# liannuaa/GenPC

Hardware: NVIDIA B200
Metric: chamfer_fwd_bwd_point_pairs_per_sec (higher is better)
Workload: dtype f32

## Files before the change

genpc_b200/csrc/chamfer.cu:

```cuda
#include <cstdlib>
#include <cstring>
#include <mutex>
#include <new>

#include "nn_core.cuh"
#include "nn_sym.cuh"
#include "nn_tc.cuh"
#include "nn_prune.cuh"
#include "nn_grid.cuh"

#ifndef GENPC_DEFAULT_SYM
#define GENPC_DEFAULT_SYM true
#endif
#ifndef GENPC_DEFAULT_PERSIST
#define GENPC_DEFAULT_PERSIST false
#endif
#ifndef GENPC_DEFAULT_BALANCED
#define GENPC_DEFAULT_BALANCED true
#endif

namespace genpc {

struct NNDir {
    const float *q;
// ... 283 lines not shown
    int cs = 1, mixed = 0;
    const char *k = tunable("GENPC_SORT_CLUSTER");
    if (k != nullptr) {
        mixed = k[0] == 'm' ? 1 : 0;
        cs = atoi(k + mixed);
        cs = cs >= 8 ? 8 : cs >= 4 ? 4 : cs == 3 ? 3 : cs == 2 ? 2 : 1;
    } else if (nmax >= 8192) {
        if (nmin * 4 <= nmax && nmin <= 4096) {
            mixed = 1;
            cs = nb * 4 + (nb + 3) / 4 * 4 <= sms ? 4 : nb * 3 + (nb + 2) / 3 * 3 <= sms ? 3 : nb * 2 + (nb + 1) / 2 * 2 <= sms ? 2 : 1;
        } else {
            cs = nb * 16 <= sms ? 8 : nb * 8 <= sms ? 4 : nb * 4 <= sms ? 2 : 1;
        }
    }
    if (cs < 2) mixed = 0;
    const int ctas = mixed ? nb * cs + nb : 2 * nb * cs;
    *mixed_out = mixed;
    *grid_out = (ctas + cs - 1) / cs * cs;
    return cs;
}

static void launch_bin_sort(PruneSortParams sp, int nb, cudaStream_t stream) {
    int mixed = 0, grid = 0;
    const int cs = sort_layout(nb, sp.n[0], sp.n[1], num_sms(), &mixed, &grid);
    sp.mixed = mixed;
    const int ctas = mixed ? nb * cs + nb : 2 * nb * cs;
    if (cs == 8) launch_bin_sort_cs<8>(sp, ctas, stream);
    else if (cs == 4) launch_bin_sort_cs<4>(sp, ctas, stream);
    else if (cs == 3) launch_bin_sort_cs<3>(sp, ctas, stream);
    else if (cs == 2) launch_bin_sort_cs<2>(sp, ctas, stream);
    else nn_bin_sort_kernel<1><<<2 * nb, PR_SORT_THREADS, 0, stream>>>(sp);
}

static int launch_prune_subbatch(const float *rows, const float *cols, int nr, int nc, unsigned long long *prow, unsigned long long *pcol,
                                 int B, int b0, int nb, int *ctl, void *prune_extra, bool accumulate, cudaStream_t stream,
                                 int *chunk_ctl = nullptr) {
    char *w = reinterpret_cast<char *>((reinterpret_cast<size_t>(prune_extra) + 255) & ~(size_t)255);
    float4 *sorted0 = reinterpret_cast<float4 *>(w);
    float4 *sorted1 = sorted0 + (size_t)B * pr_npad(nr);
    float4 *boxes0 = sorted1 + (size_t)B * pr_npad(nc);
    float4 *boxes1 = boxes0 + (size_t)B * 2 * pr_nblk(nr);
    float *bbx = reinterpret_cast<float *>(boxes1 + (size_t)B * 2 * pr_nblk(nc));
    PruneSortParams sp = {};
    sp.xyz[0] = rows + (size_t)b0 * nr * 3, sp.xyz[1] = cols + (size_t)b0 * nc * 3, sp.n[0] = nr, sp.n[1] = nc, sp.B = nb;
    sp.limit = 1e15f, sp.ctl = chunk_ctl != nullptr ? chunk_ctl : ctl, sp.hilbert = 1, sp.accumulate = accumulate ? 1 : 0;
    sp.flag = chunk_ctl != nullptr ? ctl + 1 : nullptr;
    sp.sorted[0] = sorted0 + (size_t)b0 * pr_npad(nr), sp.sorted[1] = sorted1 + (size_t)b0 * pr_npad(nc);
    sp.boxes[0] = boxes0 + (size_t)b0 * 2 * pr_nblk(nr), sp.boxes[1] = boxes1 + (size_t)b0 * 2 * pr_nblk(nc);
    sp.bbx = bbx + (size_t)b0 * 16;
    launch_bin_sort(sp, nb, stream);
    GENPC_CHECK_LAUNCH();
    PruneParams q = {};
    q.B = nb, q.select = ctl + 1, q.stats = g_prune_stats;
    q.q = sp.sorted[0], q.t = sp.sorted[1], q.tbox = sp.boxes[1], q.out = prow + (size_t)b0 * nr, q.nq = nr, q.nt = nc;
    PruneParams q2 = q;
    q2.q = sp.sorted[1], q2.t = sp.sorted[0], q2.tbox = sp.boxes[0], q2.out = pcol + (size_t)b0 * nc, q2.nq = nc, q2.nt = nr;
    launch_prune(q, q2, stream);
    GENPC_CHECK_LAUNCH();
    return GENPC_OK;
}

static int chamfer_forward_sym(const float *xyz1, const float *xyz2, float *dist1, float *dist2, int *idx1, int *idx2,
                               int B, int N, int M, unsigned long long *packed, int *counter, cudaStream_t stream,
                               const unsigned *gate = nullptr, unsigned gate_gen = 0, int gate_pairs = 1,
                               const genpc_chamfer_fuse_t *fuse = nullptr, double *fuse_partial = nullptr,
                               unsigned *fuse_ticket = nullptr, void *prune_extra = nullptr, const int *prune_chunks = nullptr) {
    const bool swap = M > N;
    SymParams p = {};
    p.rows = swap ? xyz2 : xyz1, p.cols = swap ? xyz1 : xyz2;
    p.nr = swap ? M : N, p.nc = swap ? N : M;
    float *dist_r = swap ? dist2 : dist1, *dist_c = swap ? dist1 : dist2;
    int *idx_r = swap ? idx2 : idx1, *idx_c = swap ? idx1 : idx2;
    p.prow = packed, p.pcol = packed + (size_t)B * p.nr;
    p.rblock_base = 0;
    p.gate = gate, p.gate_gen = gate_gen, p.gate_pairs = gate_pairs;
    p.select = nullptr;
    int *ctl = counter;
    const bool use_grid = ctl != nullptr && gate == nullptr && prune_extra != nullptr && B <= 8 && grid_eligible(p.nr, p.nc);
    const bool use_prune = use_grid || (ctl != nullptr && gate == nullptr && prune_extra != nullptr && prune_eligible(B, p.nr, p.nc));
    if (use_grid) {
        char *w = reinterpret_cast<char *>((reinterpret_cast<size_t>(prune_extra) + 255) & ~(size_t)255);
        GridParams gp = {};
        gp.B = B, gp.limit = 1e15f, gp.ctl = ctl;
        gp.xyz[0] = p.rows, gp.xyz[1] = p.cols, gp.n[0] = p.nr, gp.n[1] = p.nc;
        for (int i = 0; i < 2; ++i) {
            gp.sorted[i] = reinterpret_cast<float4 *>(w), w += (size_t)B * pr_npad(gp.n[i]) * sizeof(float4);
            gp.boxes[i] = reinterpret_cast<float4 *>(w), w += (size_t)B * 2 * pr_nblk(gp.n[i]) * sizeof(float4);
            gp.sboxes[i] = reinterpret_cast<float4 *>(w), w += (size_t)B * 2 * gr_nsb(gp.n[i]) * sizeof(float4);
        }
// ... 19 lines not shown
                                                                 (const int *)vals_in, vals_out, gp.n[side], 0, 30, stream);
                if (es != cudaSuccess) return (int)es;
                grid_gather_kernel<<<ctas, GR_THREADS, 0, stream>>>(gp, side, b, side == 0 && b == 0);
            }
        GENPC_CHECK_LAUNCH();
        const int nblk_max = pr_nblk(nmax), nsb_max = gr_nsb(nmax);
        grid_boxes_kernel<false><<<dim3((nblk_max + 7) / 8, B, 2), GR_THREADS, 0, stream>>>(gp);
        grid_boxes_kernel<true><<<dim3((nsb_max + 7) / 8, B, 2), GR_THREADS, 0, stream>>>(gp);
        GENPC_CHECK_LAUNCH();
        p.select = ctl + 1;
        Prune2Params q = {};
        q.B = B, q.select = ctl + 1, q.stats = g_prune_stats;
        const char *pk = tunable("GENPC_CHAMFER_PRUNE");
        const bool forced = pk != nullptr && atoi(pk) == 2;
        for (int pass = forced ? 1 : 0; pass < 2; ++pass) {
            const bool probe = pass == 0;
            long long limit = 0;
            for (int dir = 0; dir < 2; ++dir) {
                q.q = gp.sorted[dir], q.t = gp.sorted[1 - dir], q.tbox = gp.boxes[1 - dir], q.tsbox = gp.sboxes[1 - dir];
                q.out = dir == 0 ? p.prow : p.pcol, q.nq = gp.n[dir], q.nt = gp.n[1 - dir];
                const int groups = (q.nq + PR_GROUP - 1) / PR_GROUP, nblk = pr_nblk(q.nt);
                q.probe_stride = groups > GR_PROBE_GROUPS ? groups / GR_PROBE_GROUPS : 1;
                q.probe_cap = nblk / 5 > 64 ? nblk / 5 : 64;
                q.probe_acc = ctl + 2;
                const long long sampled = (long long)B * ((groups + q.probe_stride - 1) / q.probe_stride);
                limit += sampled * (nblk / 10 > 16 ? nblk / 10 : 16);
                launch_prune2(q, stream, probe);
            }
            if (probe) grid_decide_kernel<<<1, 1, 0, stream>>>(ctl, (int)(limit > 0x7fffffffLL ? 0x7fffffffLL : limit));
        }
        GENPC_CHECK_LAUNCH();
    } else if (use_prune) {
        if (prune_chunks == nullptr) {
            const int rcp = launch_prune_subbatch(p.rows, p.cols, p.nr, p.nc, p.prow, p.pcol, B, 0, B, ctl, prune_extra, false, stream);
            if (rcp != GENPC_OK) return rcp;
        } else {
            prune_rearm_kernel<<<2 * GENPC_NUM_SMS, 256, 0, stream>>>(p.prow, (size_t)B * (p.nr + p.nc), ctl + 1);
            GENPC_CHECK_LAUNCH();
        }
        p.select = ctl + 1;
    }
    const bool use_tc = !use_prune && ctl != nullptr && tc_eligible(B, p.nr, p.nc);
    if (use_tc) {
        static bool attr_done = false;
        if (!attr_done) {
            cudaError_t ea = cudaFuncSetAttribute(nn_tc_kernel<false>, cudaFuncAttributeMaxDynamicSharedMemorySize, (int)sizeof(TcSmem));
            if (ea == cudaSuccess) ea = cudaFuncSetAttribute(nn_tc_kernel<true>, cudaFuncAttributeMaxDynamicSharedMemorySize, (int)sizeof(TcSmem));
            if (ea != cudaSuccess) return (int)ea;
            attr_done = true;
        }
        const char *lim = tunable("GENPC_TC_LIMIT");
        const float limit = lim != nullptr ? (float)atof(lim) : 2.0f;
        if (gate == nullptr) {
            nn_tc_precheck_kernel<<<2 * GENPC_NUM_SMS, 256, 0, stream>>>(p.rows, (size_t)B * p.nr * 3, p.cols, (size_t)B * p.nc * 3, limit, ctl);
            GENPC_CHECK_LAUNCH();
            p.select = ctl + 1;
        }
        TcParams t = {};
        t.rows = p.rows, t.cols = p.cols, t.prow = p.prow, t.pcol = p.pcol, t.B = B, t.nr = p.nr, t.nc = p.nc;
        t.rblks = (p.nr + TC_RBLK - 1) / TC_RBLK, t.total_units = B * t.rblks;
        t.select = p.select, t.gate = gate, t.gate_gen = gate_gen, t.gate_pairs = gate_pairs, t.stats = g_tc_stats;
        const int grid = t.total_units < GENPC_NUM_SMS ? t.total_units : GENPC_NUM_SMS;
        if (gate != nullptr) nn_tc_kernel<true><<<grid, TC_THREADS, sizeof(TcSmem), stream>>>(t);
        else nn_tc_kernel<false><<<grid, TC_THREADS, sizeof(TcSmem), stream>>>(t);
        GENPC_CHECK_LAUNCH();
    }
    const bool fp32_needed = !use_tc || gate == nullptr;
    int QT = p.nr >= 1024 ? 4 : 2;
    const char *fq = tunable("GENPC_SYM_QT");
    if (gate == nullptr && fq != nullptr && (atoi(fq) == 8 || atoi(fq) == 6 || atoi(fq) == 4 || atoi(fq) == 2)) QT = atoi(fq);
    p.rtiles = (p.nr + SYM_THREADS * QT - 1) / (SYM_THREADS * QT);
    int span = SYM_SPAN_MAX;
    const long long want = 2LL * 3 * GENPC_NUM_SMS;
    while (span > 256 && (long long)B * p.rtiles * ((p.nc + span - 1) / span) < want) span >>= 1;
    const char *fs = tunable("GENPC_SYM_SPAN");
    if (fs != nullptr && atoi(fs) >= 32 && atoi(fs) <= SYM_SPAN_MAX && atoi(fs) % 32 == 0) span = atoi(fs);
    p.span = span;
    p.cspans = (p.nc + span - 1) / span;
    const long long items = (long long)B * p.rtiles * p.cspans;
    if (items > 0x7fffffffLL) return GENPC_ERR_RANGE;
    const char *pm = tunable("GENPC_SYM_PERSIST");
    const bool persist = (pm == nullptr) ? GENPC_DEFAULT_PERSIST : (atoi(pm) != 0);
    const char *bm = tunable("GENPC_SYM_BALANCED");
    const bool few_items = (long long)B * p.rtiles * ((p.nc + SYM_SPAN_MAX - 1) / SYM_SPAN_MAX) < 4LL * GENPC_NUM_SMS;
    const bool balanced = (bm == nullptr) ? ((GENPC_DEFAULT_BALANCED && few_items) || use_grid) : (atoi(bm) != 0);
    if (!fp32_needed) {
    } else if (gate != nullptr) {
        if (QT >= 4) nn_sym_gated_kernel<4><<<(unsigned)items, SYM_THREADS, 0, stream>>>(p);
        else nn_sym_gated_kernel<2><<<(unsigned)items, SYM_THREADS, 0, stream>>>(p);
    } else if (balanced && !persist && (QT == 4 || QT == 2)) {
        const int upj = (p.nc + 31) / 32;
        const long long units = (long long)B * p.rtiles * upj;
        if (units > 0x7fffffffLL) return GENPC_ERR_RANGE;
        const int grid = (int)(units < 2LL * GENPC_NUM_SMS ? units : 2LL * GENPC_NUM_SMS);
        if (QT == 4) nn_sym_balanced_kernel<4><<<grid, SYM_THREADS, 0, stream>>>(p, (int)units, upj);
        else nn_sym_balanced_kernel<2><<<grid, SYM_THREADS, 0, stream>>>(p, (int)units, upj);
#if GENPC_SYM_SPAN_MAX <= 1024
    } else if (persist && (QT == 4 || QT == 2) && counter != nullptr) {
        const int grid = (int)(items < 2LL * GENPC_NUM_SMS ? items : 2LL * GENPC_NUM_SMS);
        if (QT == 4) nn_sym_persistent_kernel<4><<<grid, SYM_THREADS, 0, stream>>>(p, (int)items, counter);
        else nn_sym_persistent_kernel<2><<<grid, SYM_THREADS, 0, stream>>>(p, (int)items, counter);
#endif
    } else if (QT == 4 && tunable("GENPC_SYM_TMA") != nullptr && atoi(tunable("GENPC_SYM_TMA")) == 1 && p.nc % 4 == 0 && p.span % 4 == 0 &&
               (reinterpret_cast<size_t>(p.cols) & 15) == 0) {
        nn_sym_tma_kernel<4><<<(unsigned)items, SYM_THREADS, 0, stream>>>(p);
    } else
    switch (QT) {
        case 8: nn_sym_kernel<8><<<(unsigned)items, SYM_THREADS, 0, stream>>>(p); break;
        case 6: nn_sym_kernel<6><<<(unsigned)items, SYM_THREADS, 0, stream>>>(p); break;
        case 4: nn_sym_kernel<4><<<(unsigned)items, SYM_THREADS, 0, stream>>>(p); break;
        default: nn_sym_kernel<2><<<(unsigned)items, SYM_THREADS, 0, stream>>>(p); break;
    }
    GENPC_CHECK_LAUNCH();
    const size_t nrw = (size_t)B * p.nr, ncw = (size_t)B * p.nc;
    const unsigned fix_blocks = (unsigned)((ncw + EPI_COLS_PER_CTA - 1) / EPI_COLS_PER_CTA);
    const unsigned unpack_blocks = (unsigned)((nrw + EPI_ROWS_PER_CTA - 1) / EPI_ROWS_PER_CTA);
    EpiFuse f;
    memset(&f, 0, sizeof(f));
    f.select = use_tc ? (gate == nullptr ? ctl + 1 : ctl + 2) : (use_prune ? ctl + 1 : nullptr);
    if (fuse == nullptr) {
        nn_sym_epilogue_kernel<false><<<fix_blocks + unpack_blocks, 256, 0, stream>>>(
            p.rows, p.cols, p.prow, p.pcol, B, p.nr, p.nc, 32 * QT, fix_blocks, dist_r, idx_r, dist_c, idx_c, f);
    } else {
        const double f1 = (fuse->w1 != 0.f) ? (double)fuse->w1 / (double)((size_t)B * N) : 0.0;
        const double f2 = (fuse->w2 != 0.f) ? (double)fuse->w2 / (double)((size_t)B * M) : 0.0;
        f.frow = swap ? f2 : f1, f.fcol = swap ? f1 : f2;
        f.use_sqrt = fuse->use_sqrt, f.rearm = 1;
        if (fuse->loss_out != nullptr) f.partial = fuse_partial, f.ticket = fuse_ticket, f.loss_out = fuse->loss_out;
        f.zero[0] = fuse->zero1, f.nzero[0] = (size_t)B * N * 3;
        f.zero[1] = fuse->zero2, f.nzero[1] = (size_t)B * M * 3;
        f.err_flag = gate != nullptr ? gate + GATE_ERR_SLOT : nullptr;
        nn_sym_epilogue_kernel<true><<<fix_blocks + unpack_blocks, 256, 0, stream>>>(
            p.rows, p.cols, p.prow, p.pcol, B, p.nr, p.nc, 32 * QT, fix_blocks, dist_r, idx_r, dist_c, idx_c, f);
    }
    GENPC_CHECK_LAUNCH();
    return GENPC_OK;
}

static size_t sym_epilogue_ctas(int B, int N, int M) {
    const size_t nr = (size_t)B * (N > M ? N : M), nc = (size_t)B * (N > M ? M : N);
    return (nc + EPI_COLS_PER_CTA - 1) / EPI_COLS_PER_CTA + (nr + EPI_ROWS_PER_CTA - 1) / EPI_ROWS_PER_CTA;
}

}

using namespace genpc;

static size_t chamfer_base_bytes(int B, int N, int M) { return ((size_t)B * N + (size_t)B * M) * sizeof(unsigned long long) + 16; }

extern "C" size_t genpc_chamfer_workspace_bytes(int B, int N, int M) {
    if (B < 0 || N < 0 || M < 0) return 0;
    return chamfer_base_bytes(B, N, M) + prune_extra_bytes(B, N, M);
// ... 255 lines not shown
    if (chunks > B) chunks = B;
    const int pairs = (B + chunks - 1) / chunks;
    chunks = (B + pairs - 1) / pairs;
    const int nr_ = M > N ? M : N, nc_ = M > N ? N : M;
    const char *hp = tunable("GENPC_HOST_PRUNE");
    if ((hp == nullptr || atoi(hp) == 1) && prune_eligible(B, nr_, nc_) && !(B <= 8 && grid_eligible(nr_, nc_)) &&
        workspace_bytes >= chamfer_base_bytes(B, N, M) + prune_extra_bytes(B, N, M)) {
        unsigned long long *packed = (unsigned long long *)workspace;
        int *ctl = (int *)(packed + n1 + n2);
        void *extra = (void *)((char *)ctl + 16);
        const float *rows = M > N ? xyz2 : xyz1, *cols = M > N ? xyz1 : xyz2;
        FEED_CHECK(cudaEventRecord(f->ready, stream));
        FEED_CHECK(cudaStreamWaitEvent(f->copy_stream, f->ready, 0));
        if (!(fuse != nullptr && fuse->workspace_armed)) {
            FEED_CHECK(cudaMemsetAsync(packed, 0xff, (n1 + n2) * 8, stream));
            FEED_CHECK(cudaMemsetAsync(ctl, 0, 16, stream));
        } else {
            FEED_CHECK(cudaMemsetAsync(ctl + 1, 0, 4, stream));
        }
        FEED_CHECK(cudaEventRecord(f->fork, stream));
        if (chunks > 2) chunks = 2;
        const int pairs = (B + chunks - 1) / chunks;
        chunks = (B + pairs - 1) / pairs;
        for (int c = 0; c < chunks; ++c) {
            const int b0 = c * pairs, nb = (B - b0 < pairs) ? B - b0 : pairs;
            if (f->cstream[c] == nullptr) FEED_CHECK(cudaStreamCreateWithFlags(&f->cstream[c], cudaStreamNonBlocking));
            FEED_CHECK(cudaMemcpyAsync(xyz1 + (size_t)b0 * N * 3, h_xyz1 + (size_t)b0 * N * 3, (size_t)nb * N * 12,
                                       cudaMemcpyHostToDevice, f->copy_stream));
            FEED_CHECK(cudaMemcpyAsync(xyz2 + (size_t)b0 * M * 3, h_xyz2 + (size_t)b0 * M * 3, (size_t)nb * M * 12,
                                       cudaMemcpyHostToDevice, f->copy_stream));
            FEED_CHECK(cudaEventRecord(f->chunk_ev[c], f->copy_stream));
            FEED_CHECK(cudaStreamWaitEvent(f->cstream[c], f->fork, 0));
            FEED_CHECK(cudaStreamWaitEvent(f->cstream[c], f->chunk_ev[c], 0));
            const int rcs = launch_prune_subbatch(rows, cols, nr_, nc_, packed, packed + (size_t)B * nr_, B, b0, nb, ctl, extra, true,
                                                  f->cstream[c], f->cctl + 4 * c);
            if (rcs != GENPC_OK) return rcs;
            FEED_CHECK(cudaEventRecord(f->done_ev[c], f->cstream[c]));
        }
        for (int c = 0; c < chunks; ++c) FEED_CHECK(cudaStreamWaitEvent(stream, f->done_ev[c], 0));
        double *partial = fuse ? (double *)fuse->loss_workspace : nullptr;
        unsigned *ticket = partial ? (unsigned *)(partial + sym_epilogue_ctas(B, N, M)) : nullptr;
        const int marker = chunks;
        return chamfer_forward_sym(xyz1, xyz2, dist1, dist2, idx1, idx2, B, N, M, packed, ctl, stream, nullptr, 0, 1, fuse, partial, ticket,
                                   extra, &marker);
    }
    const unsigned gen = ++f->gen;
    if (gen % FEED_RING == 0) FEED_CHECK(cudaEventSynchronize(f->copied));
    unsigned *src = f->h_ring + gen % FEED_RING;
    *src = gen;
    FEED_CHECK(cudaEventRecord(f->ready, stream));
    FEED_CHECK(cudaStreamWaitEvent(f->copy_stream, f->ready, 0));
    for (int c = 0; c < chunks; ++c) {
        const int b0 = c * pairs, nb = (B - b0 < pairs) ? B - b0 : pairs;
        FEED_CHECK(cudaMemcpyAsync(xyz1 + (size_t)b0 * N * 3, h_xyz1 + (size_t)b0 * N * 3, (size_t)nb * N * 12,
                                   cudaMemcpyHostToDevice, f->copy_stream));
        FEED_CHECK(cudaMemcpyAsync(xyz2 + (size_t)b0 * M * 3, h_xyz2 + (size_t)b0 * M * 3, (size_t)nb * M * 12,
                                   cudaMemcpyHostToDevice, f->copy_stream));
        FEED_CHECK(cudaMemcpyAsync(f->gate + c, src, sizeof(unsigned), cudaMemcpyHostToDevice, f->copy_stream));
    }
    unsigned long long *packed = (unsigned long long *)workspace;
    if (!(fuse != nullptr && fuse->workspace_armed)) {
        FEED_CHECK(cudaMemsetAsync(packed, 0xff, (n1 + n2) * 8, stream));
        FEED_CHECK(cudaMemsetAsync(packed + n1 + n2, 0, 16, stream));
    }
    double *partial = fuse ? (double *)fuse->loss_workspace : nullptr;
    unsigned *ticket = partial ? (unsigned *)(partial + sym_epilogue_ctas(B, N, M)) : nullptr;
    const int rc = chamfer_forward_sym(xyz1, xyz2, dist1, dist2, idx1, idx2, B, N, M, packed, (int *)(packed + n1 + n2), stream, f->gate,
// ... 187 lines not shown
```

genpc_b200/csrc/nn_prune.cuh:

```cuda
#pragma once
#include <cooperative_groups.h>

#include "common.cuh"
#include "nn_core.cuh"

#ifndef GENPC_PR_UNROLL
#define GENPC_PR_UNROLL 4
#endif

namespace genpc {

constexpr int PR_UNROLL = GENPC_PR_UNROLL;
constexpr int PR_BLOCK = 64;
constexpr int PR_GROUP = 32;
constexpr int PR_MAX_N = 32768;
constexpr int PR_SORT_THREADS = 1024;
constexpr int PR_MAX_CELLS = 4096;
constexpr int PR_THREADS = 256;

__host__ __device__ inline int pr_nblk(int n) { return (n + PR_BLOCK - 1) / PR_BLOCK; }
__host__ __device__ inline int pr_npad(int n) { return pr_nblk(n) * PR_BLOCK; }

template <int BITS>
__device__ __forceinline__ unsigned hilbert_key(unsigned x, unsigned y, unsigned z) {
// ... 13 lines not shown
        }
    }
    X[1] ^= X[0], X[2] ^= X[1];
    unsigned t = 0;
#pragma unroll
    for (unsigned Q = M; Q > 1; Q >>= 1)
        if (X[2] & Q) t ^= Q - 1;
    X[0] ^= t, X[1] ^= t, X[2] ^= t;
    unsigned key = 0;
#pragma unroll
    for (int j = BITS - 1; j >= 0; --j)
#pragma unroll
        for (int i = 0; i < 3; ++i) key = (key << 1) | ((X[i] >> j) & 1u);
    return key;
}

struct PruneSortParams {
    const float *xyz[2];
    float4 *sorted[2];
    float4 *boxes[2];
    int n[2];
    int B;
    float limit;
    int *ctl;
    int hilbert;
    float *bbx;
    int accumulate;
    int *flag;
    int side0, single_side;
    int mixed;
    int src_div[2];
    const Similarity *sim[2];
};

static __global__ void prune_rearm_kernel(unsigned long long *words, size_t n, const int *select) {
    if (*select == 0) return;
    for (size_t i = (size_t)blockIdx.x * blockDim.x + threadIdx.x; i < n; i += (size_t)gridDim.x * blockDim.x) words[i] = ~0ull;
}

template <int CS>
static __global__ void __launch_bounds__(PR_SORT_THREADS) nn_bin_sort_kernel(const PruneSortParams p) {
    __shared__ __align__(16) int hist[PR_MAX_CELLS];
    __shared__ __align__(16) int slot[CS > 1 ? PR_MAX_CELLS : 4];
    __shared__ float sred[6][PR_SORT_THREADS / 32];
    __shared__ float cbox[8];
    __shared__ int swarp[PR_SORT_THREADS / 32];
    const int tid = threadIdx.x, lane = tid & 31, warp = tid >> 5;
    int cr = 0, r0 = 0, ceff = 1, cloud = (int)blockIdx.x;
    bool idle = false;
    if constexpr (CS > 1) {
        const int rank = (int)cooperative_groups::this_cluster().block_rank();
        if (p.mixed) {
            const int big = p.n[1] > p.n[0] ? 1 : 0;
            if ((int)blockIdx.x < p.B * CS) {
                cloud = big * p.B + (int)blockIdx.x / CS, cr = rank, ceff = CS;
            } else {
                const int j = (int)blockIdx.x - p.B * CS;
                idle = j >= p.B;
                cloud = (1 - big) * p.B + (idle ? 0 : j), r0 = rank;
            }
        } else {
            cloud = (int)blockIdx.x / CS, cr = rank, ceff = CS;
        }
    }
    const int side = p.single_side ? p.side0 : cloud / p.B, b = cloud % p.B;
    const int STRIDE = ceff * PR_SORT_THREADS;
    const int n = idle ? 0 : p.n[side], nblk = pr_nblk(n), npad = nblk * PR_BLOCK;
    const float *src = p.xyz[side] + (size_t)(p.src_div[side] > 1 ? b / p.src_div[side] : b) * n * 3;
    __shared__ Similarity sT;
    const bool moved = p.sim[side] != nullptr;
    if (moved && tid == 0) sT = p.sim[side][b];
// ... 172 lines not shown
            float x, y, z;
            const int cell = cell_of(k, x, y, z);
            const int pos = atomicAdd(&next[cell], 1);
            dst[pos] = make_float4(x, y, z, __int_as_float(k));
        }
    }
    const float qnan = __int_as_float(0x7fc00000);
    if (cr == 0)
        for (int k = n + tid; k < npad; k += PR_SORT_THREADS) dst[k] = make_float4(qnan, qnan, qnan, __int_as_float(0));
    if constexpr (CS > 1) {
        __threadfence();
        cooperative_groups::this_cluster().sync();
    } else {
        __syncthreads();
    }
    for (int blk = cr * (PR_SORT_THREADS / 32) + warp; blk < nblk; blk += ceff * (PR_SORT_THREADS / 32)) {
        float l[3] = {inf, inf, inf}, h[3] = {-inf, -inf, -inf};
#pragma unroll
        for (int e = 0; e < PR_BLOCK / 32; ++e) {
            const float4 t = CS > 1 ? __ldcg(dst + blk * PR_BLOCK + e * 32 + lane) : dst[blk * PR_BLOCK + e * 32 + lane];
            l[0] = fminf(l[0], t.x), h[0] = fmaxf(h[0], t.x);
            l[1] = fminf(l[1], t.y), h[1] = fmaxf(h[1], t.y);
            l[2] = fminf(l[2], t.z), h[2] = fmaxf(h[2], t.z);
        }
#pragma unroll
        for (int c = 0; c < 3; ++c)
#pragma unroll
            for (int o = 16; o > 0; o >>= 1) {
                l[c] = fminf(l[c], __shfl_xor_sync(0xffffffffu, l[c], o));
                h[c] = fmaxf(h[c], __shfl_xor_sync(0xffffffffu, h[c], o));
            }
        if (lane == 0) bx[blk] = make_float4(l[0], l[1], l[2], 0.f), bx[nblk + blk] = make_float4(h[0], h[1], h[2], 0.f);
    }
    if (tid == 0) {
        if (anybad) atomicOr(p.ctl + 2, 1);
        __threadfence();
        if (atomicAdd(p.ctl + 3, 1) == (int)gridDim.x - 1) {
            __threadfence();
            int apart = 0;
            if (p.bbx != nullptr && !p.single_side) {
                for (int i = 0; i < p.B; ++i) {
                    const volatile float *u = p.bbx + (size_t)i * 8, *v = p.bbx + ((size_t)p.B + i) * 8;
                    float gap2 = 0.f, du = 0.f, dv = 0.f;
                    for (int c = 0; c < 3; ++c) {
                        const float g = fmaxf(fmaxf(u[c] - v[3 + c], v[c] - u[3 + c]), 0.f);
                        gap2 += g * g, du += (u[3 + c] - u[c]) * (u[3 + c] - u[c]), dv += (v[3 + c] - v[c]) * (v[3 + c] - v[c]);
                    }
                    if (gap2 > 0.0625f * fminf(du, dv)) apart = 1;
                    if (fminf(du, dv) < 0.0625f * fmaxf(du, dv)) apart = 1;
                }
            }
            const int verdict = atomicExch(p.ctl + 2, 0) | apart;
            if (p.flag != nullptr) {
                if (verdict) atomicOr(p.flag, 1);
            } else {
                p.ctl[1] = p.accumulate ? (p.ctl[1] | verdict) : verdict;
            }
            p.ctl[3] = 0;
        }
    }
}

template <int CS>
static void launch_bin_sort_cs(PruneSortParams sp, int ctas, cudaStream_t stream) {
    cudaLaunchConfig_t cfg = {};
    cfg.gridDim = dim3((unsigned)((ctas + CS - 1) / CS * CS));
    cfg.blockDim = dim3(PR_SORT_THREADS);
    cfg.stream = stream;
    cudaLaunchAttribute attr[1];
    attr[0].id = cudaLaunchAttributeClusterDimension;
    attr[0].val.clusterDim.x = CS, attr[0].val.clusterDim.y = 1, attr[0].val.clusterDim.z = 1;
    cfg.attrs = attr, cfg.numAttrs = 1;
    if (cudaLaunchKernelEx(&cfg, nn_bin_sort_kernel<CS>, sp) != cudaSuccess) {
        (void)cudaGetLastError();
        sp.mixed = 0;
        nn_bin_sort_kernel<1><<<(sp.single_side ? 1 : 2) * sp.B, PR_SORT_THREADS, 0, stream>>>(sp);
    }
}


struct PruneParams {
    const float4 *q, *t;
    const float4 *tbox;
    unsigned long long *out;
    int nq, nt, B;
    const int *select;
    unsigned *stats;
    int qdiv, tdiv;
};

__device__ __forceinline__ int pr_f2ord(float f) {
    const int i = __float_as_int(f);
    return i ^ ((i >> 31) & 0x7fffffff);
}
__device__ __forceinline__ float pr_ord2f(int i) { return __int_as_float(i ^ ((i >> 31) & 0x7fffffff)); }

struct PrunePair {
    PruneParams d[2];
    int ctas0;
    int ctas1_unused;
};

template <int BOXR>
__global__ void __launch_bounds__(PR_THREADS) nn_prune_kernel(const PrunePair pp) {
    __shared__ __align__(16) float stage[PR_THREADS / 32][3][PR_BLOCK];
    const int dir = (int)blockIdx.x >= pp.ctas0 ? 1 : 0;
    const PruneParams &p = pp.d[dir];
    if (p.select != nullptr && *p.select != 0) return;
    const int lane = threadIdx.x & 31, wid = threadIdx.x >> 5;
    const int groups = (p.nq + PR_GROUP - 1) / PR_GROUP;
    const int ctas_per_cloud = (groups + PR_THREADS / 32 - 1) / (PR_THREADS / 32);
    const int bx = (int)blockIdx.x - dir * pp.ctas0;
    const int b = bx / ctas_per_cloud;
    const int g = (bx % ctas_per_cloud) * (PR_THREADS / 32) + wid;
    if (g >= groups) return;
    const int nblk = pr_nblk(p.nt);
    const int bt = p.tdiv > 1 ? b / p.tdiv : b, bq = p.qdiv > 1 ? b / p.qdiv : b;
    const float4 *T = p.t + (size_t)bt * pr_npad(p.nt);
    const float4 *BL = p.tbox + (size_t)bt * 2 * nblk, *BH = BL + nblk;
    const float inf = __int_as_float(0x7f800000);
    const int qi = g * PR_GROUP + lane;
    const bool valid = qi < p.nq;
// ... 65 lines not shown
                tie = true;
            }
        }
        ++scanned;
        thr = pr_ord2f(__reduce_max_sync(0xffffffffu, valid ? pr_f2ord(best) : (int)0x80000000));
    }
    int bidx = 0x7fffffff;
    {
        const float4 *tc = T + bchunk * 8;
#pragma unroll
        for (int i = 0; i < 8; ++i) {
            const float4 t = __ldg(tc + i);
            const float d = sqdist_ref(q.x, q.y, q.z, t.x, t.y, t.z);
            if (d == best) bidx = min(bidx, __float_as_int(t.w));
        }
    }
    const unsigned ties = __ballot_sync(0xffffffffu, tie && valid);
    if (ties != 0u) {
        for (int blk = 0; blk < nblk; ++blk) {
            const float4 lo = __ldg(BL + blk), hi = __ldg(BH + blk);
            const float dx = fmaxf(fmaxf(lo.x - ghi[0], glo[0] - hi.x), 0.f);
            const float dy = fmaxf(fmaxf(lo.y - ghi[1], glo[1] - hi.y), 0.f);
            const float dz = fmaxf(fmaxf(lo.z - ghi[2], glo[2] - hi.z), 0.f);
            const float s = __fmul_rn(__fmaf_rn(dz, dz, __fmaf_rn(dx, dx, __fmul_rn(dy, dy))), 0.99999f);
            if (!(s <= thr)) continue;
            const float4 *tb = T + blk * PR_BLOCK;
            for (int i = 0; i < PR_BLOCK; ++i) {
                const float4 t = __ldg(tb + i);
                const float d = sqdist_ref(q.x, q.y, q.z, t.x, t.y, t.z);
                if (tie && d == best) bidx = min(bidx, __float_as_int(t.w));
            }
        }
    }
    if (valid) p.out[(size_t)b * p.nq + __float_as_int(q.w)] = pack_dist_idx(best, bidx);
    if (p.stats != nullptr && lane == 0) {
        atomicAdd(p.stats + 0, scanned);
        if (ties != 0u) atomicAdd(p.stats + 1, 1u);
        atomicAdd(p.stats + 2, 1u);
    }
}

template <int BOXR>
__global__ void __launch_bounds__(PR_THREADS) nn_prune_coop_kernel(const PruneParams p) {
    __shared__ __align__(16) float stage[PR_THREADS / 32][3][PR_BLOCK];
    __shared__ unsigned s_best[PR_GROUP];
    __shared__ float m_best[PR_THREADS / 32][PR_GROUP];
    __shared__ int m_chunk[PR_THREADS / 32][PR_GROUP], m_tie[PR_THREADS / 32][PR_GROUP];
    if (p.select != nullptr && *p.select != 0) return;
    const int lane = threadIdx.x & 31, wid = threadIdx.x >> 5;
    const int groups = (p.nq + PR_GROUP - 1) / PR_GROUP;
    const int b = (int)blockIdx.x / groups;
    const int g = (int)blockIdx.x % groups;
    if (wid == 0) s_best[lane] = 0x7f800000u;
    __syncthreads();
    const int nblk = pr_nblk(p.nt);
    const int bt = p.tdiv > 1 ? b / p.tdiv : b, bq = p.qdiv > 1 ? b / p.qdiv : b;
    const float4 *T = p.t + (size_t)bt * pr_npad(p.nt);
    const float4 *BL = p.tbox + (size_t)bt * 2 * nblk, *BH = BL + nblk;
    const float inf = __int_as_float(0x7f800000);
    const int qi = g * PR_GROUP + lane;
    const bool valid = qi < p.nq;
    const float4 q = p.q[(size_t)bq * pr_npad(p.nq) + qi];
    float glo[3], ghi[3];
    {
        const float v[3] = {q.x, q.y, q.z};
#pragma unroll
        for (int c = 0; c < 3; ++c) {
// ... 79 lines not shown
            best = mb, bchunk = mc, tie = mt;
        } else if (mb == best && mb < inf) {
            tie = tie || mt || mc != bchunk;
        }
    }
    thr = pr_ord2f(__reduce_max_sync(0xffffffffu, valid ? pr_f2ord(best) : (int)0x80000000));
    int bidx = 0x7fffffff;
    {
        const float4 *tc = T + bchunk * 8;
#pragma unroll
        for (int i = 0; i < 8; ++i) {
            const float4 t = __ldg(tc + i);
            const float d = sqdist_ref(q.x, q.y, q.z, t.x, t.y, t.z);
            if (d == best) bidx = min(bidx, __float_as_int(t.w));
        }
    }
    const unsigned ties = __ballot_sync(0xffffffffu, tie && valid);
    if (ties != 0u) {
        for (int blk = 0; blk < nblk; ++blk) {
            const float4 lo = __ldg(BL + blk), hi = __ldg(BH + blk);
            const float dx = fmaxf(fmaxf(lo.x - ghi[0], glo[0] - hi.x), 0.f);
            const float dy = fmaxf(fmaxf(lo.y - ghi[1], glo[1] - hi.y), 0.f);
            const float dz = fmaxf(fmaxf(lo.z - ghi[2], glo[2] - hi.z), 0.f);
            const float s = __fmul_rn(__fmaf_rn(dz, dz, __fmaf_rn(dx, dx, __fmul_rn(dy, dy))), 0.99999f);
            if (!(s <= thr)) continue;
            const float4 *tb = T + blk * PR_BLOCK;
            for (int i = 0; i < PR_BLOCK; ++i) {
                const float4 t = __ldg(tb + i);
                const float d = sqdist_ref(q.x, q.y, q.z, t.x, t.y, t.z);
                if (tie && d == best) bidx = min(bidx, __float_as_int(t.w));
            }
        }
    }
    if (valid) p.out[(size_t)b * p.nq + __float_as_int(q.w)] = pack_dist_idx(best, bidx);
    if (p.stats != nullptr && lane == 0) {
        atomicAdd(p.stats + 0, scanned);
        if (ties != 0u) atomicAdd(p.stats + 1, 1u);
        atomicAdd(p.stats + 2, 1u);
    }
}

}
```

genpc_b200/csrc/nn_sym.cuh:

```cuda
#pragma once
#include "nn_core.cuh"

namespace genpc {

constexpr int SYM_THREADS = 256;
#ifndef GENPC_SYM_SPAN_MAX
#define GENPC_SYM_SPAN_MAX 1024
#endif
constexpr int SYM_SPAN_MAX = GENPC_SYM_SPAN_MAX;
#ifndef GENPC_SYM_CHUNK
#define GENPC_SYM_CHUNK 8
#endif
#ifndef GENPC_SYM_REDUX
#define GENPC_SYM_REDUX 1
#endif
constexpr int SYM_CHUNK = GENPC_SYM_CHUNK;

struct SymParams {
    const float *rows;
    const float *cols;
    unsigned long long *prow;
    unsigned long long *pcol;
    int nr, nc, rtiles, cspans, span;
    int rblock_base;
// ... 419 lines not shown
            return sym_fix_column_v4(rp, cx, cy, cz, d, blk, lane);
        return sym_fix_column_t<4>(rp, nr, cx, cy, cz, d, blk, lane);
    }
    if (rows_per_block == 64) return sym_fix_column_t<2>(rp, nr, cx, cy, cz, d, blk, lane);
    int found = 0;
    for (int r0 = blk * rows_per_block; r0 < (blk + 1) * rows_per_block; r0 += 32) {
        const int j = r0 + lane;
        bool hit = false;
        if (j < nr) {
            const float dd = sqdist_ref(cx, cy, cz, __ldg(rp + (size_t)j * 3), __ldg(rp + (size_t)j * 3 + 1),
                                        __ldg(rp + (size_t)j * 3 + 2));
            hit = (dd == d);
        }
        const unsigned m = __ballot_sync(0xffffffffu, hit);
        if (m) {
            found = r0 + __ffs(m) - 1;
            break;
        }
    }
    return found;
}

struct EpiFuse {
    double *partial;
    unsigned *ticket;
    float *loss_out;
    double fcol, frow;
    int use_sqrt;
    int rearm;
    float *zero[2];
    size_t nzero[2];
    const unsigned *err_flag;
    const int *select;
};

__device__ __forceinline__ void epi_zero_fill(float *z, size_t n, size_t g, size_t total_threads) {
    if (z == nullptr) return;
    if ((reinterpret_cast<size_t>(z) & 15) == 0) {
        float4 *z4 = reinterpret_cast<float4 *>(z);
        const size_t n4 = n >> 2;
        for (size_t i = g; i < n4; i += total_threads) z4[i] = make_float4(0.f, 0.f, 0.f, 0.f);
        if (g < (n & 3)) z[(n4 << 2) + g] = 0.f;
    } else {
        for (size_t i = g; i < n; i += total_threads) z[i] = 0.f;
    }
}

constexpr int EPI_CPW = 8;
constexpr int EPI_COLS_PER_CTA = 8 * EPI_CPW;
constexpr int EPI_RPT = 8;
constexpr int EPI_ROWS_PER_CTA = 256 * EPI_RPT;

template <bool FUSED>
static __global__ void __launch_bounds__(256) nn_sym_epilogue_kernel(const float *__restrict__ rows, const float *__restrict__ cols,
                                                                     unsigned long long *__restrict__ prow,
                                                                     unsigned long long *__restrict__ pcol, int B, int nr,
                                                                     int nc, int rows_per_block, unsigned fix_blocks,
                                                                     float *__restrict__ dist_r, int *__restrict__ idx_r,
                                                                     float *__restrict__ dist_c, int *__restrict__ idx_c,
                                                                     const EpiFuse f) {
    const int lane = threadIdx.x & 31, warp = threadIdx.x >> 5;
    const bool cols_exact = f.select != nullptr && *f.select == 0;
    double term = 0.0;
    if (blockIdx.x >= fix_blocks) {
        const size_t n = (size_t)B * nr;
        const size_t i0 = (size_t)(blockIdx.x - fix_blocks) * EPI_ROWS_PER_CTA + threadIdx.x;
        unsigned long long w[EPI_RPT];
#pragma unroll
        for (int k = 0; k < EPI_RPT; ++k) {
            const size_t i = i0 + (size_t)k * 256;
            w[k] = (i < n) ? __ldcg(prow + i) : 0ull;
        }
#pragma unroll
        for (int k = 0; k < EPI_RPT; ++k) {
            const size_t i = i0 + (size_t)k * 256;
            if (i < n) {
                const float d = __uint_as_float((unsigned)(w[k] >> 32));
                dist_r[i] = d;
                idx_r[i] = (int)(unsigned)(w[k] & 0xffffffffu);
                if (FUSED) {
                    if (f.rearm) prow[i] = ~0ull;
                    term += (double)(f.use_sqrt ? __fsqrt_rn(d) : d);
                }
            }
        }
    } else {
        const size_t n = (size_t)B * nc;
        const size_t w0 = ((size_t)blockIdx.x * 8 + warp) * EPI_CPW;
        const size_t mine = w0 + (lane % EPI_CPW);
        unsigned long long my_w = 0ull;
        float mx = 0.f, my = 0.f, mz = 0.f;
        size_t my_base = 0;
        if (mine < n) {
            my_w = __ldcg(pcol + mine);
            mx = __ldg(cols + mine * 3), my = __ldg(cols + mine * 3 + 1), mz = __ldg(cols + mine * 3 + 2);
            my_base = (mine / nc) * (size_t)nr * 3;
        }
// ... 68 lines not shown
```

Baseline: 11900 billion.

## Write prune results directly to dist/idx outputs and skip packed-word epilogue

The prune kernels now store distance and index straight into the final output arrays instead of packed 64-bit words. The epilogue then only reduces the loss from those arrays when the prune result is exact. This removes the rearm kernel and the packed-word unpack traffic. It also forces the balanced sym schedule whenever pruning is used, and parallelises the bounding-box verdict in the last sort CTA across all of its threads. The risk is that the fallback path (select != 0) may still read packed words that are no longer written or rearmed, and the chunk-only fix path for the columns looks partial.

After: 12730 billion, median of 6. +7.0%, better.

```diff
diff --git a/genpc_b200/csrc/chamfer.cu b/genpc_b200/csrc/chamfer.cu
--- a/genpc_b200/csrc/chamfer.cu
+++ b/genpc_b200/csrc/chamfer.cu
@@ -339,8 +339,8 @@
     else nn_bin_sort_kernel<1><<<2 * nb, PR_SORT_THREADS, 0, stream>>>(sp);
 }
 
-static int launch_prune_subbatch(const float *rows, const float *cols, int nr, int nc, unsigned long long *prow, unsigned long long *pcol,
-                                 int B, int b0, int nb, int *ctl, void *prune_extra, bool accumulate, cudaStream_t stream,
+static int launch_prune_subbatch(const float *rows, const float *cols, int nr, int nc, float *dist_r, int *idx_r, float *dist_c,
+                                 int *idx_c, int B, int b0, int nb, int *ctl, void *prune_extra, bool accumulate, cudaStream_t stream,
                                  int *chunk_ctl = nullptr) {
     char *w = reinterpret_cast<char *>((reinterpret_cast<size_t>(prune_extra) + 255) & ~(size_t)255);
     float4 *sorted0 = reinterpret_cast<float4 *>(w);
@@ -359,9 +359,11 @@
     GENPC_CHECK_LAUNCH();
     PruneParams q = {};
     q.B = nb, q.select = ctl + 1, q.stats = g_prune_stats;
-    q.q = sp.sorted[0], q.t = sp.sorted[1], q.tbox = sp.boxes[1], q.out = prow + (size_t)b0 * nr, q.nq = nr, q.nt = nc;
+    q.q = sp.sorted[0], q.t = sp.sorted[1], q.tbox = sp.boxes[1], q.nq = nr, q.nt = nc;
+    q.dist = dist_r + (size_t)b0 * nr, q.idx = idx_r + (size_t)b0 * nr;
     PruneParams q2 = q;
-    q2.q = sp.sorted[1], q2.t = sp.sorted[0], q2.tbox = sp.boxes[0], q2.out = pcol + (size_t)b0 * nc, q2.nq = nc, q2.nt = nr;
+    q2.q = sp.sorted[1], q2.t = sp.sorted[0], q2.tbox = sp.boxes[0], q2.nq = nc, q2.nt = nr;
+    q2.dist = dist_c + (size_t)b0 * nc, q2.idx = idx_c + (size_t)b0 * nc;
     launch_prune(q, q2, stream);
     GENPC_CHECK_LAUNCH();
     return GENPC_OK;
@@ -447,11 +449,9 @@
         GENPC_CHECK_LAUNCH();
     } else if (use_prune) {
         if (prune_chunks == nullptr) {
-            const int rcp = launch_prune_subbatch(p.rows, p.cols, p.nr, p.nc, p.prow, p.pcol, B, 0, B, ctl, prune_extra, false, stream);
+            const int rcp = launch_prune_subbatch(p.rows, p.cols, p.nr, p.nc, dist_r, idx_r, dist_c, idx_c, B, 0, B, ctl, prune_extra,
+                                                  false, stream);
             if (rcp != GENPC_OK) return rcp;
-        } else {
-            prune_rearm_kernel<<<2 * GENPC_NUM_SMS, 256, 0, stream>>>(p.prow, (size_t)B * (p.nr + p.nc), ctl + 1);
-            GENPC_CHECK_LAUNCH();
         }
         p.select = ctl + 1;
     }
@@ -498,7 +498,7 @@
     const bool persist = (pm == nullptr) ? GENPC_DEFAULT_PERSIST : (atoi(pm) != 0);
     const char *bm = tunable("GENPC_SYM_BALANCED");
     const bool few_items = (long long)B * p.rtiles * ((p.nc + SYM_SPAN_MAX - 1) / SYM_SPAN_MAX) < 4LL * GENPC_NUM_SMS;
-    const bool balanced = (bm == nullptr) ? ((GENPC_DEFAULT_BALANCED && few_items) || use_grid) : (atoi(bm) != 0);
+    const bool balanced = (bm == nullptr) ? ((GENPC_DEFAULT_BALANCED && few_items) || use_prune) : (atoi(bm) != 0);
     if (!fp32_needed) {
     } else if (gate != nullptr) {
         if (QT >= 4) nn_sym_gated_kernel<4><<<(unsigned)items, SYM_THREADS, 0, stream>>>(p);
@@ -533,6 +533,7 @@
     EpiFuse f;
     memset(&f, 0, sizeof(f));
     f.select = use_tc ? (gate == nullptr ? ctl + 1 : ctl + 2) : (use_prune ? ctl + 1 : nullptr);
+    f.direct = use_prune && !use_grid;
     if (fuse == nullptr) {
         nn_sym_epilogue_kernel<false><<<fix_blocks + unpack_blocks, 256, 0, stream>>>(
             p.rows, p.cols, p.prow, p.pcol, B, p.nr, p.nc, 32 * QT, fix_blocks, dist_r, idx_r, dist_c, idx_c, f);
@@ -854,7 +855,8 @@
             FEED_CHECK(cudaEventRecord(f->chunk_ev[c], f->copy_stream));
             FEED_CHECK(cudaStreamWaitEvent(f->cstream[c], f->fork, 0));
             FEED_CHECK(cudaStreamWaitEvent(f->cstream[c], f->chunk_ev[c], 0));
-            const int rcs = launch_prune_subbatch(rows, cols, nr_, nc_, packed, packed + (size_t)B * nr_, B, b0, nb, ctl, extra, true,
+            const int rcs = launch_prune_subbatch(rows, cols, nr_, nc_, M > N ? dist2 : dist1, M > N ? idx2 : idx1,
+                                                  M > N ? dist1 : dist2, M > N ? idx1 : idx2, B, b0, nb, ctl, extra, true,
                                                   f->cstream[c], f->cctl + 4 * c);
             if (rcs != GENPC_OK) return rcs;
             FEED_CHECK(cudaEventRecord(f->done_ev[c], f->cstream[c]));
diff --git a/genpc_b200/csrc/nn_prune.cuh b/genpc_b200/csrc/nn_prune.cuh
--- a/genpc_b200/csrc/nn_prune.cuh
+++ b/genpc_b200/csrc/nn_prune.cuh
@@ -69,11 +69,6 @@
     int src_div[2];
     const Similarity *sim[2];
 };
-
-static __global__ void prune_rearm_kernel(unsigned long long *words, size_t n, const int *select) {
-    if (*select == 0) return;
-    for (size_t i = (size_t)blockIdx.x * blockDim.x + threadIdx.x; i < n; i += (size_t)gridDim.x * blockDim.x) words[i] = ~0ull;
-}
 
 template <int CS>
 static __global__ void __launch_bounds__(PR_SORT_THREADS) nn_bin_sort_kernel(const PruneSortParams p) {
@@ -312,24 +307,30 @@
             }
         if (lane == 0) bx[blk] = make_float4(l[0], l[1], l[2], 0.f), bx[nblk + blk] = make_float4(h[0], h[1], h[2], 0.f);
     }
+    __shared__ int s_last;
     if (tid == 0) {
         if (anybad) atomicOr(p.ctl + 2, 1);
         __threadfence();
-        if (atomicAdd(p.ctl + 3, 1) == (int)gridDim.x - 1) {
-            __threadfence();
-            int apart = 0;
-            if (p.bbx != nullptr && !p.single_side) {
-                for (int i = 0; i < p.B; ++i) {
-                    const volatile float *u = p.bbx + (size_t)i * 8, *v = p.bbx + ((size_t)p.B + i) * 8;
-                    float gap2 = 0.f, du = 0.f, dv = 0.f;
-                    for (int c = 0; c < 3; ++c) {
-                        const float g = fmaxf(fmaxf(u[c] - v[3 + c], v[c] - u[3 + c]), 0.f);
-                        gap2 += g * g, du += (u[3 + c] - u[c]) * (u[3 + c] - u[c]), dv += (v[3 + c] - v[c]) * (v[3 + c] - v[c]);
-                    }
-                    if (gap2 > 0.0625f * fminf(du, dv)) apart = 1;
-                    if (fminf(du, dv) < 0.0625f * fmaxf(du, dv)) apart = 1;
+        s_last = atomicAdd(p.ctl + 3, 1) == (int)gridDim.x - 1;
+    }
+    __syncthreads();
+    if (s_last) {
+        __threadfence();
+        int apart = 0;
+        if (p.bbx != nullptr && !p.single_side) {
+            for (int i = tid; i < p.B; i += PR_SORT_THREADS) {
+                const volatile float *u = p.bbx + (size_t)i * 8, *v = p.bbx + ((size_t)p.B + i) * 8;
+                float gap2 = 0.f, du = 0.f, dv = 0.f;
+                for (int c = 0; c < 3; ++c) {
+                    const float g = fmaxf(fmaxf(u[c] - v[3 + c], v[c] - u[3 + c]), 0.f);
+                    gap2 += g * g, du += (u[3 + c] - u[c]) * (u[3 + c] - u[c]), dv += (v[3 + c] - v[c]) * (v[3 + c] - v[c]);
                 }
-            }
+                if (gap2 > 0.0625f * fminf(du, dv)) apart = 1;
+                if (fminf(du, dv) < 0.0625f * fmaxf(du, dv)) apart = 1;
+            }
+        }
+        apart = __syncthreads_or(apart);
+        if (tid == 0) {
             const int verdict = atomicExch(p.ctl + 2, 0) | apart;
             if (p.flag != nullptr) {
                 if (verdict) atomicOr(p.flag, 1);
@@ -363,11 +364,19 @@
     const float4 *q, *t;
     const float4 *tbox;
     unsigned long long *out;
+    float *dist;
+    int *idx;
     int nq, nt, B;
     const int *select;
     unsigned *stats;
     int qdiv, tdiv;
 };
+
+__device__ __forceinline__ void pr_store(const PruneParams &p, int b, int orig, float best, int bidx) {
+    const size_t o = (size_t)b * p.nq + orig;
+    if (p.dist != nullptr) p.dist[o] = best, p.idx[o] = bidx;
+    else p.out[o] = pack_dist_idx(best, bidx);
+}
 
 __device__ __forceinline__ int pr_f2ord(float f) {
     const int i = __float_as_int(f);
@@ -499,7 +508,7 @@
             }
         }
     }
-    if (valid) p.out[(size_t)b * p.nq + __float_as_int(q.w)] = pack_dist_idx(best, bidx);
+    if (valid) pr_store(p, b, __float_as_int(q.w), best, bidx);
     if (p.stats != nullptr && lane == 0) {
         atomicAdd(p.stats + 0, scanned);
         if (ties != 0u) atomicAdd(p.stats + 1, 1u);
@@ -645,7 +654,7 @@
             }
         }
     }
-    if (valid) p.out[(size_t)b * p.nq + __float_as_int(q.w)] = pack_dist_idx(best, bidx);
+    if (valid) pr_store(p, b, __float_as_int(q.w), best, bidx);
     if (p.stats != nullptr && lane == 0) {
         atomicAdd(p.stats + 0, scanned);
         if (ties != 0u) atomicAdd(p.stats + 1, 1u);
diff --git a/genpc_b200/csrc/nn_sym.cuh b/genpc_b200/csrc/nn_sym.cuh
--- a/genpc_b200/csrc/nn_sym.cuh
+++ b/genpc_b200/csrc/nn_sym.cuh
@@ -475,6 +475,7 @@
     size_t nzero[2];
     const unsigned *err_flag;
     const int *select;
+    int direct;
 };
 
 __device__ __forceinline__ void epi_zero_fill(float *z, size_t n, size_t g, size_t total_threads) {
@@ -504,8 +505,26 @@
                                                                      const EpiFuse f) {
     const int lane = threadIdx.x & 31, warp = threadIdx.x >> 5;
     const bool cols_exact = f.select != nullptr && *f.select == 0;
+    const bool done = f.direct && cols_exact;
     double term = 0.0;
-    if (blockIdx.x >= fix_blocks) {
+    if (done) {
+        if (FUSED && f.partial != nullptr && blockIdx.x >= fix_blocks) {
+            const size_t n = (size_t)B * nr;
+            const size_t i0 = (size_t)(blockIdx.x - fix_blocks) * EPI_ROWS_PER_CTA + threadIdx.x;
+            float d[EPI_RPT];
+#pragma unroll
+            for (int k = 0; k < EPI_RPT; ++k) {
+                const size_t i = i0 + (size_t)k * 256;
+                d[k] = (i < n) ? dist_r[i] : 0.f;
+            }
+#pragma unroll
+            for (int k = 0; k < EPI_RPT; ++k)
+                if (i0 + (size_t)k * 256 < n) term += (double)(f.use_sqrt ? __fsqrt_rn(d[k]) : d[k]);
+        } else if (FUSED && f.partial != nullptr) {
+            const size_t mine = ((size_t)blockIdx.x * 8 + warp) * EPI_CPW + (lane % EPI_CPW);
+            if (lane < EPI_CPW && mine < (size_t)B * nc) term = (double)(f.use_sqrt ? __fsqrt_rn(dist_c[mine]) : dist_c[mine]);
+        }
+    } else if (blockIdx.x >= fix_blocks) {
         const size_t n = (size_t)B * nr;
         const size_t i0 = (size_t)(blockIdx.x - fix_blocks) * EPI_ROWS_PER_CTA + threadIdx.x;
         unsigned long long w[EPI_RPT];
```
